# ugadiarov-la-phystech-edu/OCRL

Hardware: AMD Instinct MI355X
Metric: images/sec (node) SLATE pretrain 128x128, 6 slots, 3 iters (higher is better)
Workload: dtype f32

## Files before the change

ocrl_amd/csrc/slot_attn.hip:

```cpp
#include "common.h"
#include "kernels.h"

#define SA_C 64
#include <stdlib.h>
#define SA_TF 1024
#define SA_TB 512
#define SA_TLD 68
#define SA_WLD 17
#define SA_MAX_BLOCKS 2048

typedef float f32x4_t __attribute__((ext_vector_type(4)));
#define MFMA16(a, b, c) __builtin_amdgcn_mfma_f32_16x16x4f32((a), (b), (c), 0, 0, 0)

__device__ inline float sigmoidf_(float x) { return 1.0f / (1.0f + __expf(-x)); }
#define SA_ROR(v, n) __builtin_bit_cast(float, __builtin_amdgcn_update_dpp(0, __builtin_bit_cast(int, (v)), 0x120 + (n), 0xF, 0xF, false))
__device__ inline float red16_sum(float v) {
    v += SA_ROR(v, 8); v += SA_ROR(v, 4); v += SA_ROR(v, 2); v += SA_ROR(v, 1);
    return v;
}
__device__ inline float red16_max(float v) {
    v = fmaxf(v, SA_ROR(v, 8)); v = fmaxf(v, SA_ROR(v, 4)); v = fmaxf(v, SA_ROR(v, 2)); v = fmaxf(v, SA_ROR(v, 1));
    return v;
}
__device__ inline float redg_sum(float v) {
// ... 601 lines not shown
            for (int c = 0; c < 4; ++c) od[c] = pos0 < N ? dxb[pos0 * 16 + 4 * c + g] : make_float4(0.f, 0.f, 0.f, 0.f);
        }
        f32x4_t L = (f32x4_t){l0, l0, l0, l0}, DA = (f32x4_t){d0, d0, d0, d0};
#pragma unroll
        for (int k = 0; k < 16; ++k) { L = MFMA16(xn[k], qpr[k], L); DA = MFMA16(xn[k], dur[k], DA); }
#pragma unroll
        for (int c = 0; c < 4; ++c)
            *reinterpret_cast<float4*>(tile + li * SA_TLD + 16 * c + 4 * g) = make_float4(xn[4 * c], xn[4 * c + 1], xn[4 * c + 2], xn[4 * c + 3]);
        f32x4_t dl, wn;
#pragma unroll
        for (int r = 0; r < 4; ++r) {
            const float x = li < K ? L[r] : -INFINITY;
            const float mx = red16_max(x);
            const float e = li < K ? __expf(x - mx) : 0.f;
            const float a = e / red16_sum(e);
            const float da = (DA[r] - udv) * icv;
            const float dot = red16_sum(a * da);
            const bool ok = li < K && (t * 16 + 4 * g + r) < N;
            dl[r] = ok ? a * (da - dot) : 0.f;
            wn[r] = ok ? (a + eps) * icv : 0.f;
            sdl += dl[r];
            wt0[(4 * g + r) * SA_WLD + li] = wn[r];
            wt1[(4 * g + r) * SA_WLD + li] = dl[r];
        }
        __builtin_amdgcn_wave_barrier();
#pragma unroll
        for (int r = 0; r < 4; ++r)
#pragma unroll
            for (int m = 0; m < 4; ++m) acc[m] = MFMA16(tile[(4 * g + r) * SA_TLD + 16 * m + li], dl[r], acc[m]);
        f32x4_t Dx[4];
#pragma unroll
        for (int m = 0; m < 4; ++m) Dx[m] = (f32x4_t){0.f, 0.f, 0.f, 0.f};
#pragma unroll
        for (int s = 0; s < NS; ++s) {
            const float wa = wt0[li * SA_WLD + 4 * s + g], da2 = wt1[li * SA_WLD + 4 * s + g];
#pragma unroll
            for (int m = 0; m < 4; ++m) { Dx[m] = MFMA16(wa, duB[s][m], Dx[m]); Dx[m] = MFMA16(da2, qpB[s][m], Dx[m]); }
        }
        __builtin_amdgcn_wave_barrier();
#pragma unroll
        for (int m = 0; m < 4; ++m)
#pragma unroll
            for (int r = 0; r < 4; ++r) tile[(4 * g + r) * SA_TLD + 16 * m + li] = Dx[m][r];
        __builtin_amdgcn_wave_barrier();
        float dv[16];
#pragma unroll
        for (int c = 0; c < 4; ++c) {
            const float4 d4 = *reinterpret_cast<const float4*>(tile + li * SA_TLD + 16 * c + 4 * g);
            dv[4 * c] = d4.x; dv[4 * c + 1] = d4.y; dv[4 * c + 2] = d4.z; dv[4 * c + 3] = d4.w;
        }
        __builtin_amdgcn_wave_barrier();
        const int pos = t * 16 + li;
        if (!FIRST) {
#pragma unroll
            for (int c = 0; c < 4; ++c) { dv[4 * c] += od[c].x; dv[4 * c + 1] += od[c].y; dv[4 * c + 2] += od[c].z; dv[4 * c + 3] += od[c].w; }
        }
        if (FINAL) {
            float m1 = 0.f, m2 = 0.f;
#pragma unroll
            for (int k = 0; k < 16; ++k) { m1 += dv[k]; m2 += dv[k] * xn[k]; }
            m1 = redg_sum(m1) * (1.0f / SA_C);
            m2 = redg_sum(m2) * (1.0f / SA_C);
#pragma unroll
            for (int k = 0; k < 16; ++k) dv[k] = rs * (dv[k] - m1 - xn[k] * m2);
        }
        if (pos < N) {
#pragma unroll
            for (int c = 0; c < 4; ++c) dxb[pos * 16 + 4 * c + g] = make_float4(dv[4 * c], dv[4 * c + 1], dv[4 * c + 2], dv[4 * c + 3]);
        }
#pragma unroll
        for (int c = 0; c < 4; ++c) cur[c] = nxt[c];
    }
    sdl = redg_sum(sdl);
    __syncthreads();
    if (li < K) {
#pragma unroll
        for (int m = 0; m < 4; ++m)
#pragma unroll
            for (int r = 0; r < 4; ++r) scr[(wv * K + li) * (SA_C + 1) + 16 * m + 4 * g + r] = acc[m][r];
        if (g == 0) scr[(wv * K + li) * (SA_C + 1) + SA_C] = sdl;
    }
}

template <int K, bool FIRST, bool FINAL>
__device__ __forceinline__ void sa_stream_bwd2(const float4* __restrict__ xb, float4* __restrict__ dxb, int N, const float* qg, const float* qb,
                                               const float* dug, const float* dub, const float* cs, const float* ud, float eps, float* tiles,
                                               float* scr, int tile0, int tile1) {
    const int tid = threadIdx.x, lane = tid & 63, wv = tid >> 6, nw = blockDim.x >> 6, li = lane & 15, g = lane >> 4;
    float* tile = tiles + wv * (16 * SA_TLD + 2 * 16 * SA_WLD);
    float* wt = tile + 16 * SA_TLD;
    float qpr[16], dur[16];
#pragma unroll
    for (int k = 0; k < 16; ++k) {
        const int ch = 16 * (k >> 2) + 4 * g + (k & 3);
        qpr[k] = li < K ? qg[li * SA_C + ch] * SA_LOG2E : 0.f;
        dur[k] = li < K ? dug[li * SA_C + ch] : 0.f;
    }
    float duA[4][4], qgA[4][4];
#pragma unroll
    for (int m = 0; m < 4; ++m)
#pragma unroll
        for (int r = 0; r < 4; ++r) {
            const int slot = 4 * g + r;
            duA[m][r] = slot < K ? dug[slot * SA_C + 16 * m + li] : 0.f;
            qgA[m][r] = slot < K ? qg[slot * SA_C + 16 * m + li] : 0.f;
        }
    float qbr[4], dbr[4], icr[4];
#pragma unroll
    for (int r = 0; r < 4; ++r) {
        const int slot = 4 * g + r;
        qbr[r] = slot < K ? qb[slot] * SA_LOG2E : -1e30f;
        icr[r] = slot < K ? 1.0f / cs[slot] : 0.f;
        dbr[r] = slot < K ? dub[slot] - ud[slot] : 0.f;
    }
    f32x4_t acc[4];
#pragma unroll
    for (int m = 0; m < 4; ++m) acc[m] = (f32x4_t){0.f, 0.f, 0.f, 0.f};
    float sdl[4] = {0.f, 0.f, 0.f, 0.f};
    const int ntile = tile1;
    float4 cur[4];
    if (tile0 + wv < ntile) sa_load_tile(xb, N, tile0 + wv, li, g, cur);
#pragma unroll 1
    for (int t = tile0 + wv; t < ntile; t += nw) {
        float4 nxt[4];
        if (t + nw < ntile) sa_load_tile(xb, N, t + nw, li, g, nxt);
        const int pos = t * 16 + li;
        float4 od[4];
        if (!FIRST) {
#pragma unroll
            for (int c = 0; c < 4; ++c) od[c] = pos < N ? dxb[pos * 16 + 4 * c + g] : make_float4(0.f, 0.f, 0.f, 0.f);
        }
        f32x2_t v2[8];
#pragma unroll
        for (int c = 0; c < 4; ++c) { v2[2 * c] = (f32x2_t){cur[c].x, cur[c].y}; v2[2 * c + 1] = (f32x2_t){cur[c].z, cur[c].w}; }
        f32x2_t s2 = ((v2[0] + v2[1]) + (v2[2] + v2[3])) + ((v2[4] + v2[5]) + (v2[6] + v2[7]));
        const float mu = sa_xrow_sum4(s2.x + s2.y) * (1.0f / SA_C);
        const f32x2_t mu2 = (f32x2_t){mu, mu};
#pragma unroll
        for (int k = 0; k < 8; ++k) v2[k] -= mu2;
        f32x2_t q2 = v2[0] * v2[0];
#pragma unroll
        for (int k = 1; k < 8; ++k) q2 = __builtin_elementwise_fma(v2[k], v2[k], q2);
        const float rs = __builtin_amdgcn_rsqf(sa_xrow_sum4(q2.x + q2.y) * (1.0f / SA_C) + 1e-5f);
        f32x4_t La = (f32x4_t){0.f, 0.f, 0.f, 0.f}, Lb = La, Da = La, Db = La;
#pragma unroll
        for (int k = 0; k < 8; ++k) {
            La = MFMA16(qpr[2 * k], v2[k].x, La);
            Da = MFMA16(dur[2 * k], v2[k].x, Da);
            Lb = MFMA16(qpr[2 * k + 1], v2[k].y, Lb);
            Db = MFMA16(dur[2 * k + 1], v2[k].y, Db);
        }
#pragma unroll
        for (int c = 0; c < 4; ++c)
            *reinterpret_cast<float4*>(tile + li * SA_TLD + 16 * c + 4 * g) = make_float4(v2[2 * c].x, v2[2 * c].y, v2[2 * c + 1].x, v2[2 * c + 1].y);
        float l[4];
#pragma unroll
        for (int r = 0; r < 4; ++r) l[r] = __builtin_fmaf(La[r] + Lb[r], rs, qbr[r]);
        float mx = fmaxf(fmaxf(l[0], l[1]), fmaxf(l[2], l[3]));
        mx = sa_xrow16(mx, true);
        if (K > 8) mx = sa_xrow32(mx, true);
        float a[4];
#pragma unroll
        for (int r = 0; r < 4; ++r) a[r] = __builtin_amdgcn_exp2f(l[r] - mx);
        float sm = (a[0] + a[1]) + (a[2] + a[3]);
        sm = sa_xrow16(sm, false);
        if (K > 8) sm = sa_xrow32(sm, false);
        const float inv = __builtin_amdgcn_rcpf(sm);
        float da[4], dot = 0.f;
#pragma unroll
        for (int r = 0; r < 4; ++r) {
            a[r] *= inv;
            da[r] = (__builtin_fmaf(Da[r] + Db[r], rs, dbr[r])) * icr[r];
            dot = __builtin_fmaf(a[r], da[r], dot);
        }
        dot = sa_xrow16(dot, false);
        if (K > 8) dot = sa_xrow32(dot, false);
        const float live = pos < N ? 1.f : 0.f;
        float dl[4], wn[4];
#pragma unroll
        for (int r = 0; r < 4; ++r) {
            dl[r] = a[r] * (da[r] - dot) * live;
            wn[r] = (a[r] + eps) * icr[r] * live;
            sdl[r] += dl[r];
            wt[(4 * g + r) * SA_WT_LD + li] = dl[r] * rs;
        }
        __builtin_amdgcn_wave_barrier();
        const float4 wb4 = *reinterpret_cast<const float4*>(wt + li * SA_WT_LD + 4 * g);
        const float wb[4] = {wb4.x, wb4.y, wb4.z, wb4.w};
#pragma unroll
        for (int r = 0; r < 4; ++r)
#pragma unroll
            for (int m = 0; m < 4; ++m) acc[m] = MFMA16(tile[(4 * g + r) * SA_TLD + 16 * m + li], wb[r], acc[m]);
        f32x4_t Dx[4];
#pragma unroll
        for (int m = 0; m < 4; ++m) Dx[m] = (f32x4_t){0.f, 0.f, 0.f, 0.f};
#pragma unroll
        for (int r = 0; r < 4; ++r)
#pragma unroll
            for (int m = 0; m < 4; ++m) {
                Dx[m] = MFMA16(duA[m][r], wn[r], Dx[m]);
                Dx[m] = MFMA16(qgA[m][r], dl[r], Dx[m]);
            }
        __builtin_amdgcn_wave_barrier();
        float dv[16];
#pragma unroll
        for (int m = 0; m < 4; ++m) { dv[4 * m] = Dx[m][0]; dv[4 * m + 1] = Dx[m][1]; dv[4 * m + 2] = Dx[m][2]; dv[4 * m + 3] = Dx[m][3]; }
        if (!FIRST) {
#pragma unroll
            for (int c = 0; c < 4; ++c) { dv[4 * c] += od[c].x; dv[4 * c + 1] += od[c].y; dv[4 * c + 2] += od[c].z; dv[4 * c + 3] += od[c].w; }
        }
        if (FINAL) {
            float m1 = 0.f, m2 = 0.f;
#pragma unroll
            for (int k = 0; k < 8; ++k) {
                m1 += dv[2 * k] + dv[2 * k + 1];
                m2 += dv[2 * k] * v2[k].x + dv[2 * k + 1] * v2[k].y;
            }
            m1 = sa_xrow_sum4(m1) * (1.0f / SA_C);
            m2 = sa_xrow_sum4(m2) * rs * (1.0f / SA_C);
#pragma unroll
            for (int k = 0; k < 8; ++k) {
                dv[2 * k] = rs * (dv[2 * k] - m1 - v2[k].x * rs * m2);
                dv[2 * k + 1] = rs * (dv[2 * k + 1] - m1 - v2[k].y * rs * m2);
            }
        }
        if (pos < N) {
#pragma unroll
            for (int c = 0; c < 4; ++c) dxb[pos * 16 + 4 * c + g] = make_float4(dv[4 * c], dv[4 * c + 1], dv[4 * c + 2], dv[4 * c + 3]);
        }
#pragma unroll
        for (int c = 0; c < 4; ++c) cur[c] = nxt[c];
    }
#pragma unroll
    for (int r = 0; r < 4; ++r) sdl[r] = red16_sum(sdl[r]);
    __syncthreads();
    if (li < K) {
#pragma unroll
        for (int m = 0; m < 4; ++m)
#pragma unroll
            for (int r = 0; r < 4; ++r) scr[(wv * K + li) * (SA_C + 1) + 16 * m + 4 * g + r] = acc[m][r];
    }
    if (li == 0) {
#pragma unroll
        for (int r = 0; r < 4; ++r)
            if (4 * g + r < K) scr[(wv * K + 4 * g + r) * (SA_C + 1) + SA_C] = sdl[r];
    }
}

template <int K, int G>
struct SaBwdLds {
    float *ds, *t2, *t0, *t1, *dgi, *dgh, *dhid, *qp, *dup, *dqp, *qg, *dug, *cs, *ud, *qb, *dub, *sdl, *gacc;
    __device__ SaBwdLds(float* sm, int D, int H, int NH) {
        constexpr int C = SA_C, KB = SaGeo<K, G>::KB, KP = SaGeo<K, G>::KP;
        const int KV = NH * KP;
        ds = sm;
        t2 = ds + KP * D;
        t0 = t2 + KP * D;
        t1 = t0 + KB * D;
        dgi = t1 + KB * D;
        dgh = dgi + KB * 3 * D;
        dhid = dgh + KB * 3 * D;
        qp = dhid + KB * H;
        dup = qp + KV * C;
        dqp = dup + KV * C;
        qg = dqp + KV * C;
        dug = qg + KV * C;
        cs = dug + KV * C;
        ud = cs + 16;
        qb = ud + 16;
        dub = qb + 16;
        sdl = dub + 16;
        gacc = sdl + 16;
    }
};

template <int K, int G>
__device__ __forceinline__ void sa_bwd_part1(const SaBwdLds<K, G>& L, const SlotAttnArgs& p, const SaWts& wo, const SaSave& so, const SaGrad& go,
                                             const SaRowMap& sv, const SaRowMap& gr, int nvalid) {
    constexpr int C = SA_C, NB = SaGeo<K, G>::NB, KB = SaGeo<K, G>::KB, KP = SaGeo<K, G>::KP;
    const int D = p.D, H = p.H, tid = threadIdx.x, nt = blockDim.x, NH = p.NH, dh = D / NH, KV = NH * KP;
    const float* W = p.wts;
    float* dg_m = L.gacc + 2 * D;  float* db_m = L.gacc + 3 * D;
#pragma unroll 1
    for (int hb = 0; hb < NB; ++hb) {
        const int j0 = hb * KB, kv = (nvalid - j0) < KB ? (nvalid - j0 > 0 ? nvalid - j0 : 0) : KB;
// ... 38 lines not shown
#pragma unroll 1
        for (int h = 0; h < NH; ++h)
            matvec<KB>(W + wo.WvT, D / 16, 0, h * dh / 16, dh, C, t1 + h * dh, D, L.dup + (h * KP + j0) * C, C, nullptr, 1.f);
    }
    for (int h = 0; h < NH; ++h) rows_get(L.qp + h * KP * C, sv, so.qp + h * C, 0, nvalid, C);
    for (int i = tid; i < KV * C; i += nt)
        if (((i >> 6) % KP) >= nvalid) { L.qp[i] = 0.f; L.dup[i] = 0.f; }
    __syncthreads();
    if (tid < KV) {
        const int h = tid / KP, r = tid - h * KP;
        if (r < nvalid) {
            const float* row = sv(r);
            L.cs[tid] = row[so.csum + h];
            float a = 0.f;
            for (int c = 0; c < C; ++c) a += row[so.up + h * C + c] * L.dup[tid * C + c];
            L.ud[tid] = a;
        }
    }
    __syncthreads();
    sa_fold_affine(L.qp, W + wo.ln_in_g, W + wo.ln_in_b, L.qg, L.qb, KV);
    sa_fold_affine(L.dup, W + wo.ln_in_g, W + wo.ln_in_b, L.dug, L.dub, KV);
    __syncthreads();
}

template <int K, int G>
__device__ __forceinline__ void sa_bwd_part2(const SaBwdLds<K, G>& L, const SlotAttnArgs& p, const SaWts& wo, const SaSave& so, const SaGrad& go,
                                             const SaRowMap& sv, const SaRowMap& gr, int b0, int NS, int nvalid) {
    constexpr int C = SA_C, NB = SaGeo<K, G>::NB, KB = SaGeo<K, G>::KB, KP = SaGeo<K, G>::KP;
    const int D = p.D, tid = threadIdx.x, nt = blockDim.x, NH = p.NH, dh = D / NH, KV = NH * KP;
    const float* W = p.wts;
    float* dg_s = L.gacc;  float* db_s = L.gacc + D;
    float* dg_in = L.gacc + 4 * D;  float* db_in = L.gacc + 4 * D + C;
    float *dqp = L.dqp, *sdl = L.sdl, *t0 = L.t0, *t1 = L.t1;
    const int pstride = NH * K * (C + 1);
    if (tid < KV) {
        const int h = tid / KP, r = tid - h * KP;
        sdl[tid] = r < nvalid ? sa_psum(p.parts + (size_t)(b0 + r / K) * NS * pstride, NS, pstride, (h * K + r % K) * (C + 1) + C) : 0.f;
    }
    for (int i = tid; i < KV * C; i += nt) {
        const int v = i >> 6, c = i & 63, h = v / KP, r = v - h * KP;
        dqp[i] = r < nvalid ? sa_psum(p.parts + (size_t)(b0 + r / K) * NS * pstride, NS, pstride, (h * K + r % K) * (C + 1) + c) : 0.f;
    }
    __syncthreads();
    if (tid < C) {
        float dg = 0.f, db = 0.f;
        for (int h = 0; h < NH; ++h)
            for (int r = 0; r < nvalid; ++r) {
                const int j = h * KP + r;
                dg += L.dup[j * C + tid] * sv(r)[so.upn + h * C + tid] + L.qp[j * C + tid] * dqp[j * C + tid];
                db += L.dup[j * C + tid] + L.qp[j * C + tid] * sdl[j];
            }
        dg_in[tid] += dg;
        db_in[tid] += db;
    }
    __syncthreads();
    for (int i = tid; i < KV * C; i += nt) {
        const int j = i >> 6, c = i & 63;
        if ((j % KP) < nvalid) dqp[i] = dqp[i] * W[wo.ln_in_g + c] + W[wo.ln_in_b + c] * sdl[j];
    }
    __syncthreads();
    for (int h = 0; h < NH; ++h) rows_put(dqp + h * KP * C, gr, go.qp + h * C, 0, nvalid, C);
#pragma unroll 1
    for (int hb = 0; hb < NB; ++hb) {
        const int j0 = hb * KB, kv = (nvalid - j0) < KB ? (nvalid - j0 > 0 ? nvalid - j0 : 0) : KB;
        float* dsB = L.ds + j0 * D;
#pragma unroll 1
        for (int h = 0; h < NH; ++h)
            matvec<KB>(W + wo.Wk, C / 16, h * dh / 16, 0, C, dh, dqp + (h * KP + j0) * C, C, t1 + h * dh, D, nullptr, p.scale);
        rows_put(t1, gr, go.q, j0, kv, D);
        rows_get(t0, sv, so.sprev, j0, kv, D);
        for (int i = kv * D + tid; i < KB * D; i += nt) t0[i] = 0.f;
        matvec<KB>(W + wo.WqT, D / 16, 0, 0, D, D, t1, D, dsB, D, nullptr, 1.f);
        for (int i = tid; i < kv * D; i += nt) { t1[i] = dsB[i]; dsB[i] = L.t2[j0 * D + i]; }
        __syncthreads();
        ln_rows_bwd(t1, t0, dsB, 1, W + wo.ln_s_g, dg_s, db_s, kv, D);
        __syncthreads();
    }
}

__host__ __device__ inline size_t sa_xchg_bwd_floats(int K, int D) {
    const int KI = K > 8 ? 2 * ((K + 1) / 2) : K;
    return ((size_t)KI * D + 3 * (size_t)KI * SA_C + 64 + 15) & ~(size_t)15;
}
template <int K, int G>
__global__ __launch_bounds__(SA_TB) void sa_slot_bwd_kernel(SlotAttnArgs p, SaWts wo, SaSave so, SaGrad go, int t_hi, int t_lo, int NS) {
    extern __shared__ __attribute__((aligned(16))) float sm[];
    const int D = p.D;
    constexpr int C = SA_C, KP = SaGeo<K, G>::KP;
    const int nt = blockDim.x, tid = threadIdx.x, NH = p.NH, KV = NH * KP, KI = sa_ki(NH * K);
    const SaBwdLds<K, G> L(sm, D, p.H, NH);
    const int b0 = blockIdx.x * G;
    const int nimg = (p.B - b0) < G ? (p.B - b0) : G, nvalid = nimg * K;
    const size_t XF = sa_xchg_bwd_floats(NH * K, D);
    float* xg0 = p.xchg + (size_t)b0 * XF;
    const int SM = 4 * D + 2 * C;
    float* gs = p.g_small + (size_t)b0 * SM;
    if (t_hi < 0) {
        for (int i = tid; i < KP * D; i += nt) L.ds[i] = i < nvalid * D ? p.dslots[(size_t)b0 * K * D + i] : 0.f;
        for (int i = tid; i < SM; i += nt) L.gacc[i] = 0.f;
    } else {
        for (int i = tid; i < KP * D; i += nt) { const int r = i / D, c = i - r * D; L.t2[i] = r < nvalid ? xg0[(size_t)(r / K) * XF + (r % K) * D + c] : 0.f; }
        for (int i = tid; i < KV * C; i += nt) {
            const int v = i >> 6, c = i & 63, h = v / KP, r = v - h * KP;
            L.dup[i] = r < nvalid ? xg0[(size_t)(r / K) * XF + KI * D + (h * K + r % K) * C + c] : 0.f;
        }
        for (int i = tid; i < SM; i += nt) L.gacc[i] = gs[i];
        for (int h = 0; h < NH; ++h) rows_get(L.qp + h * KP * C, sa_rows(p.save, so.ld, b0, t_hi, p.I, K), so.qp + h * C, 0, nvalid, C);
        for (int i = tid; i < KV * C; i += nt)
            if (((i >> 6) % KP) >= nvalid) L.qp[i] = 0.f;
    }
    __syncthreads();
    if (t_hi >= 0)
        sa_bwd_part2<K, G>(L, p, wo, so, go, sa_rows(p.save, so.ld, b0, t_hi, p.I, K), sa_rows(p.grows, go.ld, b0, t_hi, p.I, K), b0, NS, nvalid);
    if (t_lo >= 0) {
        sa_bwd_part1<K, G>(L, p, wo, so, go, sa_rows(p.save, so.ld, b0, t_lo, p.I, K), sa_rows(p.grows, go.ld, b0, t_lo, p.I, K), nvalid);
        for (int i = tid; i < nvalid * D; i += nt) { const int r = i / D, c = i - r * D; xg0[(size_t)(r / K) * XF + (r % K) * D + c] = L.t2[i]; }
        for (int i = tid; i < KV * C; i += nt) {
            const int v = i >> 6, c = i & 63, h = v / KP, r = v - h * KP;
            if (r >= nvalid) continue;
            float* x = xg0 + (size_t)(r / K) * XF + KI * D + (h * K + r % K) * C + c;
            x[0] = L.dup[i]; x[KI * C] = L.qg[i]; x[2 * KI * C] = L.dug[i];
        }
        if (tid < KV) {
            const int h = tid / KP, r = tid - h * KP;
            if (r < nvalid) {
                float* x = xg0 + (size_t)(r / K) * XF + KI * D + 3 * KI * C + h * K + r % K;
                x[0] = L.qb[tid]; x[16] = L.dub[tid]; x[32] = L.cs[tid]; x[48] = L.ud[tid];
            }
        }
    } else {
        for (int i = tid; i < nvalid * D; i += nt) p.dslots0[(size_t)b0 * K * D + i] = L.ds[i];
    }
    for (int i = tid; i < SM; i += nt) gs[i] = L.gacc[i];
    for (int i = tid; i < (nimg - 1) * SM; i += nt) gs[SM + i] = 0.f;
}
template <int K, bool FIRST, bool FINAL, bool V2>
__global__ __launch_bounds__(SA_TS, 2) void sa_stream_bwd_kernel(SlotAttnArgs p, int NS) {
    extern __shared__ __attribute__((aligned(16))) float sm[];
    constexpr int C = SA_C, KP = SaBlk<K>::KP;
    const int D = p.D, N = p.N, nt = blockDim.x, nw = nt >> 6, tid = threadIdx.x;
    float* qg = sm;
    float* dug = qg + KP * C;
    float* sv4 = dug + KP * C;
    float* tiles = sv4 + 64;
    const int b = blockIdx.x / NS, h = blockIdx.x % NS;
    const float* xg = p.xchg + (size_t)b * sa_xchg_bwd_floats(K, D);
    const float *g_qg = xg + KP * D + KP * C, *g_dug = g_qg + KP * C, *g_small4 = g_dug + KP * C;
    for (int i = tid; i < K * C; i += nt) { qg[i] = g_qg[i]; dug[i] = g_dug[i]; }
    if (tid < 64) sv4[tid] = g_small4[tid];
    __syncthreads();
    const float4* xb = reinterpret_cast<const float4*>(p.x + (size_t)b * N * C);
    float4* dxb = reinterpret_cast<float4*>(p.dx + (size_t)b * N * C);
    const int ntile = (N + 15) / 16, per = (ntile + NS - 1) / NS;
    const int t0 = h * per, t1 = (t0 + per < ntile) ? t0 + per : ntile;
    if (V2) sa_stream_bwd2<K, FIRST, FINAL>(xb, dxb, N, qg, sv4, dug, sv4 + 16, sv4 + 32, sv4 + 48, p.eps, tiles, tiles, t0, t1 > t0 ? t1 : t0);
    else sa_stream_bwd<K, FIRST, FINAL>(xb, dxb, N, qg, sv4, dug, sv4 + 16, sv4 + 32, sv4 + 48, p.eps, tiles, tiles, t0, t1 > t0 ? t1 : t0);
    __syncthreads();
    float* part = p.parts + ((size_t)b * NS + h) * K * (C + 1);
    for (int i = tid; i < K * (C + 1); i += nt) {
        float a = 0.f;
        for (int w = 0; w < nw; ++w) a += tiles[w * K * (C + 1) + i];
        part[i] = a;
    }
}

static size_t sa_fwd_smem(int K, int G, int D, int H, int NH = 1) {
    const int NB = K > 8 ? 2 : 1, KB = K > 8 ? (K + 1) / 2 : G * K, KP = NB * KB;
    return (size_t)(KP * D + KB * D * 3 + KB * 3 * D * 2 + KB * H + NH * KP * SA_C * 3 + 32) * 4;
}
static size_t sa_bwd_smem(int K, int G, int D, int H, int NH = 1) {
    const int NB = K > 8 ? 2 : 1, KB = K > 8 ? (K + 1) / 2 : G * K, KP = NB * KB;
    return (size_t)(KP * D * 2 + KB * D * 2 + KB * 3 * D * 2 + KB * H + NH * KP * SA_C * 5 + 80 + 4 * D + 2 * SA_C) * 4;
}
#define SA_LDS_MAX (160 * 1024 - 256)
int sa_plan(int K, int D, int H, int NH, SaPlan* pl) {
    OCRL_REQUIRE(K >= 1 && K <= 16, "slot_attn: 1 <= num_slots <= 16 supported (got %d)", K);
    OCRL_REQUIRE(D > 0 && H > 0 && D % 64 == 0 && H % 64 == 0 && D <= 256 && H <= 256,
                 "slot_attn: slot/mlp size must be multiples of 64, <= 256 (got %d / %d)", D, H);
    OCRL_REQUIRE(NH >= 1 && D % NH == 0, "slot_attn: the slot size %d does not divide into %d heads", D, NH);
    if (NH > 1)
        OCRL_REQUIRE(K <= 8 && NH * K <= 16 && (D / NH) % 16 == 0,
                     "slot_attn: with %d heads, heads * num_slots <= 16 and a head width that is a multiple of 16 are supported (num_slots %d, slot size %d)", NH, K, D);
    int G = 1;
    if (NH == 1 && K <= 8 && 16 / K > 1) {
        static int gmode = -1;
        if (gmode < 0) { const char* e = getenv("OCRL_SA_GROUP"); gmode = e ? atoi(e) : 1; }
        const int GM = 16 / K;
        if (gmode && sa_fwd_smem(K, GM, D, H) <= SA_LDS_MAX && sa_bwd_smem(K, GM, D, H) <= SA_LDS_MAX) G = GM;
    }
    pl->G = G; pl->NB = K > 8 ? 2 : 1; pl->KB = K > 8 ? (K + 1) / 2 : G * K; pl->KS = NH * K;
    pl->smem_fwd = sa_fwd_smem(K, G, D, H, NH); pl->smem_bwd = sa_bwd_smem(K, G, D, H, NH);
    OCRL_REQUIRE(pl->smem_fwd <= SA_LDS_MAX && pl->smem_bwd <= SA_LDS_MAX, "slot_attn: LDS request %zu / %zu too large (num_slots %d, heads %d, slot size %d, mlp size %d)",
                 pl->smem_fwd, pl->smem_bwd, K, NH, D, H);
    return 0;
}
size_t sa_xchg_floats_host(int K, int D) {
    const size_t f = sa_xchg_floats(K, D), g = sa_xchg_bwd_floats(K, D);
    return f > g ? f : g;
}
size_t sa_parts_floats_host(int B, int K) { return (size_t)(SA_MAX_BLOCKS + B) * K * (SA_C + 1); }

static int sa_splits(int B, int N, int per_cu) {
    static int ncu = 0, mult = 0;
    if (!ncu) {
        int dev = 0;
        hipDeviceProp_t prop;
        ncu = (hipGetDevice(&dev) == hipSuccess && hipGetDeviceProperties(&prop, dev) == hipSuccess) ? prop.multiProcessorCount : 256;
        const char* e = getenv("OCRL_SA_WGS");
        mult = e ? atoi(e) : 0;
    }
    const int ntile = (N + 15) / 16;
    int target = (mult > 0 ? mult : per_cu) * ncu;
    if (target > SA_MAX_BLOCKS) target = SA_MAX_BLOCKS;
    int ns = B <= target ? target / B : 1;
    if (const char* f = getenv("OCRL_SA_NS")) { const int v = atoi(f); if (v > 0 && (long long)B * v <= SA_MAX_BLOCKS) ns = v; }
    if (ns > ntile / 8) ns = ntile / 8;
    return ns < 1 ? 1 : ns;
}

template <int K, int G>
static int sa_launch_kg(const SlotAttnArgs& a, const SaPlan& pl, int backward, hipStream_t st) {
    constexpr int KP = SaBlk<K>::KP;
    static_assert(SaGeo<K, G>::NB == (K > 8 ? 2 : 1) && SaGeo<K, G>::KB == (K > 8 ? (K + 1) / 2 : G * K), "sa_plan states the kernels' geometry");
    const size_t smem = backward ? pl.smem_bwd : pl.smem_fwd;
    static_assert((SA_TS / 64) * 16 * SA_TLD >= (SA_TS / 64) * 16 * (SA_C + 1), "streaming workgroup: partial scratch must fit the tile region");
    const SaWts wo = sa_wts_layout(a.C, a.D, a.H);
    const SaSave so = sa_save_layout(a.C, a.D, a.H);
    const SaGrad go = sa_grad_layout(a.C, a.D, a.H);
    static size_t attr_f = 0, attr_b = 0;
    if (!backward && smem > attr_f) {
        OCRL_HIP(hipFuncSetAttribute((const void*)sa_slot_fwd_kernel<K, G>, hipFuncAttributeMaxDynamicSharedMemorySize, (int)smem));
        attr_f = smem;
    }
    if (backward && smem > attr_b) {
        OCRL_HIP(hipFuncSetAttribute((const void*)sa_slot_bwd_kernel<K, G>, hipFuncAttributeMaxDynamicSharedMemorySize, (int)smem));
        attr_b = smem;
    }
    static int fwd_form = -1;
    if (fwd_form < 0) { const char* e = getenv("OCRL_SA_FWD"); fwd_form = e ? atoi(e) : 2; }
    const int NS = sa_splits(a.B, a.N, backward ? 4 : (fwd_form == 1 ? 3 : 4));
    const int ngrp = (a.B + G - 1) / G;
    const int pi = prof_begin(backward ? PROF_SA_BWD : PROF_SA_FWD, st);
    if (!backward) {
        const size_t smem_stream = (size_t)(KP * SA_C + 16 + (SA_TS / 64) * (16 * SA_TLD + 16 * SA_WT_LD)) * 4;
        if (a.phase != 2) hipLaunchKernelGGL((sa_slot_fwd_kernel<K, G>), dim3(ngrp), dim3(SA_TF), smem, st, a, wo, so, -1, NS);
        for (int t = 0; t < a.I && a.phase != 1; ++t) {
            if (fwd_form == 1) hipLaunchKernelGGL((sa_stream_fwd_kernel<K, false>), dim3(a.B * NS), dim3(SA_TS), smem_stream, st, a, t, NS);
            else hipLaunchKernelGGL((sa_stream_fwd_kernel<K, true>), dim3(a.B * NS), dim3(SA_TS), smem_stream, st, a, t, NS);
            hipLaunchKernelGGL((sa_slot_fwd_kernel<K, G>), dim3(ngrp), dim3(SA_TF), smem, st, a, wo, so, t, NS);
        }
    } else {
        static int bwd_form = -1;
        if (bwd_form < 0) { const char* e = getenv("OCRL_SA_BWD"); bwd_form = e ? atoi(e) : 2; }
        static_assert(16 * SA_WT_LD <= 2 * 16 * SA_WLD, "the weight patch of the second form must fit the first form's two patches");
        const size_t smem_stream = (size_t)(2 * KP * SA_C + 64 + (SA_TS / 64) * (16 * SA_TLD + 2 * 16 * SA_WLD)) * 4;
        hipLaunchKernelGGL((sa_slot_bwd_kernel<K, G>), dim3(ngrp), dim3(SA_TB), smem, st, a, wo, so, go, -1, a.I - 1, NS);
        for (int t = a.I - 1; t >= 0; --t) {
            const bool first = (t == a.I - 1), final_ = (t == 0);
            if (bwd_form == 1) {
                if (first && final_) hipLaunchKernelGGL((sa_stream_bwd_kernel<K, true, true, false>), dim3(a.B * NS), dim3(SA_TS), smem_stream, st, a, NS);
                else if (first) hipLaunchKernelGGL((sa_stream_bwd_kernel<K, true, false, false>), dim3(a.B * NS), dim3(SA_TS), smem_stream, st, a, NS);
                else if (final_) hipLaunchKernelGGL((sa_stream_bwd_kernel<K, false, true, false>), dim3(a.B * NS), dim3(SA_TS), smem_stream, st, a, NS);
                else hipLaunchKernelGGL((sa_stream_bwd_kernel<K, false, false, false>), dim3(a.B * NS), dim3(SA_TS), smem_stream, st, a, NS);
            } else {
                if (first && final_) hipLaunchKernelGGL((sa_stream_bwd_kernel<K, true, true, true>), dim3(a.B * NS), dim3(SA_TS), smem_stream, st, a, NS);
                else if (first) hipLaunchKernelGGL((sa_stream_bwd_kernel<K, true, false, true>), dim3(a.B * NS), dim3(SA_TS), smem_stream, st, a, NS);
                else if (final_) hipLaunchKernelGGL((sa_stream_bwd_kernel<K, false, true, true>), dim3(a.B * NS), dim3(SA_TS), smem_stream, st, a, NS);
                else hipLaunchKernelGGL((sa_stream_bwd_kernel<K, false, false, true>), dim3(a.B * NS), dim3(SA_TS), smem_stream, st, a, NS);
            }
            hipLaunchKernelGGL((sa_slot_bwd_kernel<K, G>), dim3(ngrp), dim3(SA_TB), smem, st, a, wo, so, go, t, t - 1, NS);
        }
    }
    prof_end(pi, st);
    OCRL_CHECK_LAUNCH("slot_attn");
    return 0;
}
typedef void (*SaStreamFwdFn)(SlotAttnArgs, int, int);
typedef void (*SaStreamBwdFn)(SlotAttnArgs, int);
template <int KS> static SaStreamBwdFn sa_stream_bwd_pick(bool first, bool final_) {
    if (first && final_) return sa_stream_bwd_kernel<KS, true, true, true>;
    if (first) return sa_stream_bwd_kernel<KS, true, false, true>;
    if (final_) return sa_stream_bwd_kernel<KS, false, true, true>;
    return sa_stream_bwd_kernel<KS, false, false, true>;
}
static SaStreamFwdFn sa_stream_fwd_fn(int KS) {
    switch (KS) {
#define SA_CASE(k) case k: return sa_stream_fwd_kernel<k, true>;
        SA_CASE(2) SA_CASE(3) SA_CASE(4) SA_CASE(5) SA_CASE(6) SA_CASE(7) SA_CASE(8) SA_CASE(9) SA_CASE(10) SA_CASE(11) SA_CASE(12) SA_CASE(13) SA_CASE(14) SA_CASE(15) SA_CASE(16)
#undef SA_CASE
    }
    return nullptr;
}
static SaStreamBwdFn sa_stream_bwd_fn(int KS, bool first, bool final_) {
    switch (KS) {
#define SA_CASE(k) case k: return sa_stream_bwd_pick<k>(first, final_);
        SA_CASE(2) SA_CASE(3) SA_CASE(4) SA_CASE(5) SA_CASE(6) SA_CASE(7) SA_CASE(8) SA_CASE(9) SA_CASE(10) SA_CASE(11) SA_CASE(12) SA_CASE(13) SA_CASE(14) SA_CASE(15) SA_CASE(16)
#undef SA_CASE
    }
    return nullptr;
}
__global__ void sa_attn_heads_sum_kernel(const float* __restrict__ in, float* __restrict__ out, long long rows, int K, int NH) {
    const long long n = rows * K;
    for (long long i = (long long)blockIdx.x * blockDim.x + threadIdx.x; i < n; i += (long long)gridDim.x * blockDim.x) {
        const long long r = i / K; const int k = (int)(i - r * K);
        float a = 0.f;
        for (int h = 0; h < NH; ++h) a += in[r * (NH * K) + h * K + k];
        out[i] = a;
    }
}
template <int K>
static int sa_launch_heads(const SlotAttnArgs& a0, const SaPlan& pl, int backward, hipStream_t st) {
    const int NH = a0.NH, KS = pl.KS, KPS = sa_ki(KS);
    const size_t smem = backward ? pl.smem_bwd : pl.smem_fwd;
    OCRL_REQUIRE(!a0.attn || a0.attn_heads, "slot_attn: the per-head attention scratch is missing");
    SlotAttnArgs a = a0;
    if (a.attn) a.attn = a0.attn_heads;
    const SaWts wo = sa_wts_layout(a.C, a.D, a.H);
    const SaSave so = sa_save_layout(a.C, a.D, a.H, NH);
    const SaGrad go = sa_grad_layout(a.C, a.D, a.H, NH);
    OCRL_HIP(hipFuncSetAttribute((const void*)(backward ? (const void*)sa_slot_bwd_kernel<K, 1> : (const void*)sa_slot_fwd_kernel<K, 1>),
                                 hipFuncAttributeMaxDynamicSharedMemorySize, (int)SA_LDS_MAX));
    const int NS = sa_splits(a.B, a.N, 4);
    const int pi = prof_begin(backward ? PROF_SA_BWD : PROF_SA_FWD, st);
    if (!backward) {
        const size_t smem_stream = (size_t)(KPS * SA_C + 16 + (SA_TS / 64) * (16 * SA_TLD + 16 * SA_WT_LD)) * 4;
        const SaStreamFwdFn fs = sa_stream_fwd_fn(KS);
        if (a.phase != 2) hipLaunchKernelGGL((sa_slot_fwd_kernel<K, 1>), dim3(a.B), dim3(SA_TF), smem, st, a, wo, so, -1, NS);
        for (int t = 0; t < a.I && a.phase != 1; ++t) {
            hipLaunchKernelGGL(fs, dim3(a.B * NS), dim3(SA_TS), smem_stream, st, a, t, NS);
            hipLaunchKernelGGL((sa_slot_fwd_kernel<K, 1>), dim3(a.B), dim3(SA_TF), smem, st, a, wo, so, t, NS);
        }
        if (a0.attn && a.phase != 1) {
            const long long rows = (long long)a.B * a.N;
            hipLaunchKernelGGL(sa_attn_heads_sum_kernel, dim3(cdiv(rows * K, 256) > 4096 ? 4096 : cdiv(rows * K, 256)), dim3(256), 0, st, a0.attn_heads, a0.attn, rows, K, NH);
        }
    } else {
        const size_t smem_stream = (size_t)(2 * KPS * SA_C + 64 + (SA_TS / 64) * (16 * SA_TLD + 2 * 16 * SA_WLD)) * 4;
        hipLaunchKernelGGL((sa_slot_bwd_kernel<K, 1>), dim3(a.B), dim3(SA_TB), smem, st, a, wo, so, go, -1, a.I - 1, NS);
        for (int t = a.I - 1; t >= 0; --t) {
            hipLaunchKernelGGL(sa_stream_bwd_fn(KS, t == a.I - 1, t == 0), dim3(a.B * NS), dim3(SA_TS), smem_stream, st, a, NS);
            hipLaunchKernelGGL((sa_slot_bwd_kernel<K, 1>), dim3(a.B), dim3(SA_TB), smem, st, a, wo, so, go, t, t - 1, NS);
        }
    }
    prof_end(pi, st);
    OCRL_CHECK_LAUNCH("slot_attn (heads)");
    return 0;
}

template <int K>
static int sa_launch_k(const SlotAttnArgs& a, const SaPlan& pl, int backward, hipStream_t st) {
    OCRL_REQUIRE(a.xchg && a.parts, "slot_attn: exchange / partial buffers missing");
    constexpr int GM = K <= 8 ? 16 / K : 1;
    if (GM > 1 && pl.G == GM) return sa_launch_kg<K, GM>(a, pl, backward, st);
    return sa_launch_kg<K, 1>(a, pl, backward, st);
}

int slot_attn_launch(const SlotAttnArgs& a, int backward, hipStream_t st) {
    OCRL_REQUIRE(a.C == SA_C, "slot_attn: input width must be %d (got %d)", SA_C, a.C);
    SaPlan pl;
    RC(sa_plan(a.K, a.D, a.H, a.NH, &pl));
    OCRL_REQUIRE(a.B > 0 && a.N > 0 && a.I >= 1, "slot_attn: empty problem");
    OCRL_REQUIRE((long long)a.N * 16 < (1ll << 31), "slot_attn: N too large for 32-bit row offsets");
    OCRL_REQUIRE(a.x && a.wts && ((uintptr_t)a.x & 15) == 0, "slot_attn: x/wts missing or x not 16-byte aligned");
    if (backward) OCRL_REQUIRE(a.dx && ((uintptr_t)a.dx & 15) == 0 && a.save && a.grows && a.dslots && a.dslots0 && a.g_small, "slot_attn bwd: missing buffers");
    else OCRL_REQUIRE(a.slots0 && a.slots, "slot_attn fwd: missing buffers");
    OCRL_REQUIRE(a.xchg && a.parts && ((uintptr_t)a.xchg & 15) == 0, "slot_attn: exchange / partial buffers missing or xchg not 16-byte aligned");
    if (a.NH > 1) {
        switch (a.K) {
#define SA_CASE(k) case k: return sa_launch_heads<k>(a, pl, backward, st);
            SA_CASE(1) SA_CASE(2) SA_CASE(3) SA_CASE(4) SA_CASE(5) SA_CASE(6) SA_CASE(7) SA_CASE(8)
#undef SA_CASE
        }
        return -1;
    }
    switch (a.K) {
#define SA_CASE(k) case k: return sa_launch_k<k>(a, pl, backward, st);
        SA_CASE(1) SA_CASE(2) SA_CASE(3) SA_CASE(4) SA_CASE(5) SA_CASE(6) SA_CASE(7) SA_CASE(8)
        SA_CASE(9) SA_CASE(10) SA_CASE(11) SA_CASE(12) SA_CASE(13) SA_CASE(14) SA_CASE(15) SA_CASE(16)
#undef SA_CASE
    }
    return -1;
}

__global__ void pack_kernel(const PackEntry* __restrict__ ent, float* __restrict__ dst) {
    const PackEntry e = ent[blockIdx.y];
    const int n = e.rows * e.cols;
    for (int i = blockIdx.x * blockDim.x + threadIdx.x; i < n; i += gridDim.x * blockDim.x) {
        if (e.transpose >= 2) {
            const int Et = e.transpose == 2 ? e.cols : e.rows, nks = Et >> 4;
            const int j = i & 3, lane = (i >> 2) & 63, rest = i >> 8, s = rest % nks, tile = rest / nks;
            const int col = tile * 16 + (lane & 15), k = s * 16 + (lane >> 4) * 4 + j;
            dst[e.dst_off + i] = e.transpose == 2 ? e.src[col * Et + k] : e.src[k * e.cols + col];
        } else if (e.transpose) {
            const int c = i / e.rows, r = i - c * e.rows;
            dst[e.dst_off + i] = e.src[r * e.cols + c];
        } else {
            dst[e.dst_off + i] = e.src[i];
        }
    }
}
int pack_launch(const PackEntry* entries_dev, int n_entries, int max_elems, float* dst, hipStream_t st) {
    int gx = cdiv(max_elems, 256);
    if (gx > 64) gx = 64;
    hipLaunchKernelGGL(pack_kernel, dim3(gx, n_entries), dim3(256), 0, st, entries_dev, dst);
    OCRL_CHECK_LAUNCH("pack");
    return 0;
}
```

Before: 1748.

## Defer slot-attention input gradient by recording per-iteration weights and replaying at end

Adds a new default backward form (OCRL_SA_BWD=3) for slot attention. Non-final iteration stream kernels no longer build and accumulate the full 64-channel dx per position. They store only compact per-slot attention weights (wn, dl) into the dx buffer, and the slot backward kernel saves that iteration's dug/qg into a history area. The final stream kernel reads those records and replays every iteration's contribution with extra MFMAs against the history held in LDS. This cuts dx read-modify-write traffic across iterations, at the cost of more LDS, extra MFMA work in the final pass, and a larger exchange buffer.

After: 1753 (median of 6 runs). About the same (+0.2%).

```diff
diff --git a/ocrl_amd/csrc/slot_attn.hip b/ocrl_amd/csrc/slot_attn.hip
--- a/ocrl_amd/csrc/slot_attn.hip
+++ b/ocrl_amd/csrc/slot_attn.hip
@@ -707,10 +707,24 @@
     }
 }
 
-template <int K, bool FIRST, bool FINAL>
+template <int K> struct SaRec {
+    static constexpr int NG = K > 8 ? 4 : 2;
+    static constexpr int Q = 2 * NG * 16;
+    static constexpr int MAXE = 256 / Q;
+    static constexpr int PER = K > 8 ? 1 : 2;
+    static constexpr int HOP = 2 * SA_C * SA_WT_LD;
+};
+template <int K>
+__device__ __forceinline__ int sa_rec_idx(bool whole, int j, int which, int g, int li) {
+    constexpr int NG = SaRec<K>::NG;
+    return whole ? j * SaRec<K>::Q + (which * NG + g) * 16 + li : li * 16 + j * 2 * NG + which * NG + g;
+}
+template <int K, bool FIRST, bool FINAL, bool REC = false>
 __device__ __forceinline__ void sa_stream_bwd2(const float4* __restrict__ xb, float4* __restrict__ dxb, int N, const float* qg, const float* qb,
                                                const float* dug, const float* dub, const float* cs, const float* ud, float eps, float* tiles,
-                                               float* scr, int tile0, int tile1) {
+                                               float* scr, int tile0, int tile1, int rec = 0, const float* hop = nullptr) {
+    static_assert(!REC || FIRST, "the record form never accumulates through dx");
+    constexpr bool DXN = !REC || FINAL;
     const int tid = threadIdx.x, lane = tid & 63, wv = tid >> 6, nw = blockDim.x >> 6, li = lane & 15, g = lane >> 4;
     float* tile = tiles + wv * (16 * SA_TLD + 2 * 16 * SA_WLD);
     float* wt = tile + 16 * SA_TLD;
@@ -722,14 +736,16 @@
         dur[k] = li < K ? dug[li * SA_C + ch] : 0.f;
     }
     float duA[4][4], qgA[4][4];
-#pragma unroll
-    for (int m = 0; m < 4; ++m)
-#pragma unroll
-        for (int r = 0; r < 4; ++r) {
-            const int slot = 4 * g + r;
-            duA[m][r] = slot < K ? dug[slot * SA_C + 16 * m + li] : 0.f;
-            qgA[m][r] = slot < K ? qg[slot * SA_C + 16 * m + li] : 0.f;
-        }
+    if (DXN) {
+#pragma unroll
+        for (int m = 0; m < 4; ++m)
+#pragma unroll
+            for (int r = 0; r < 4; ++r) {
+                const int slot = 4 * g + r;
+                duA[m][r] = slot < K ? dug[slot * SA_C + 16 * m + li] : 0.f;
+                qgA[m][r] = slot < K ? qg[slot * SA_C + 16 * m + li] : 0.f;
+            }
+    }
     float qbr[4], dbr[4], icr[4];
 #pragma unroll
     for (int r = 0; r < 4; ++r) {
@@ -743,6 +759,8 @@
     for (int m = 0; m < 4; ++m) acc[m] = (f32x4_t){0.f, 0.f, 0.f, 0.f};
     float sdl[4] = {0.f, 0.f, 0.f, 0.f};
     const int ntile = tile1;
+    constexpr int RPER = SaRec<K>::PER;
+    const int ngrp = REC && FINAL ? (rec + RPER - 1) / RPER : 0, ge = RPER == 2 ? g >> 1 : 0, gs = RPER == 2 ? g & 1 : g;
     float4 cur[4];
     if (tile0 + wv < ntile) sa_load_tile(xb, N, tile0 + wv, li, g, cur);
 #pragma unroll 1
@@ -750,6 +768,17 @@
         float4 nxt[4];
         if (t + nw < ntile) sa_load_tile(xb, N, t + nw, li, g, nxt);
         const int pos = t * 16 + li;
+        const bool whole = t * 16 + 16 <= N;
+        float4 rw[SaRec<K>::MAXE / RPER], rd[SaRec<K>::MAXE / RPER];
+        if (REC && FINAL) {
+#pragma unroll
+            for (int gi = 0; gi < SaRec<K>::MAXE / RPER; ++gi) {
+                const int j = gi * RPER + ge;
+                const bool have = gi < ngrp && j < rec && pos < N;
+                rw[gi] = have ? dxb[t * 256 + sa_rec_idx<K>(whole, j, 0, gs, li)] : make_float4(0.f, 0.f, 0.f, 0.f);
+                rd[gi] = have ? dxb[t * 256 + sa_rec_idx<K>(whole, j, 1, gs, li)] : make_float4(0.f, 0.f, 0.f, 0.f);
+            }
+        }
         float4 od[4];
         if (!FIRST) {
 #pragma unroll
@@ -816,6 +845,16 @@
         for (int r = 0; r < 4; ++r)
 #pragma unroll
             for (int m = 0; m < 4; ++m) acc[m] = MFMA16(tile[(4 * g + r) * SA_TLD + 16 * m + li], wb[r], acc[m]);
+        if (!DXN) {
+            __builtin_amdgcn_wave_barrier();
+            if (g < SaRec<K>::NG && pos < N) {
+                dxb[t * 256 + sa_rec_idx<K>(whole, rec, 0, g, li)] = make_float4(wn[0], wn[1], wn[2], wn[3]);
+                dxb[t * 256 + sa_rec_idx<K>(whole, rec, 1, g, li)] = make_float4(dl[0], dl[1], dl[2], dl[3]);
+            }
+#pragma unroll
+            for (int c = 0; c < 4; ++c) cur[c] = nxt[c];
+            continue;
+        }
         f32x4_t Dx[4];
 #pragma unroll
         for (int m = 0; m < 4; ++m) Dx[m] = (f32x4_t){0.f, 0.f, 0.f, 0.f};
@@ -826,6 +865,25 @@
                 Dx[m] = MFMA16(duA[m][r], wn[r], Dx[m]);
                 Dx[m] = MFMA16(qgA[m][r], dl[r], Dx[m]);
             }
+        if (REC) {
+#pragma unroll
+            for (int gi = 0; gi < SaRec<K>::MAXE / RPER; ++gi) {
+                if (gi >= ngrp) break;
+                const float* ha = hop + gi * SaRec<K>::HOP + li * SA_WT_LD + 4 * g;
+                const float bw[4] = {rw[gi].x, rw[gi].y, rw[gi].z, rw[gi].w}, bd[4] = {rd[gi].x, rd[gi].y, rd[gi].z, rd[gi].w};
+#pragma unroll
+                for (int m = 0; m < 4; ++m) {
+                    const float4 au = *reinterpret_cast<const float4*>(ha + 16 * m * SA_WT_LD);
+                    const float4 aq = *reinterpret_cast<const float4*>(ha + (SA_C + 16 * m) * SA_WT_LD);
+                    const float ua[4] = {au.x, au.y, au.z, au.w}, qa[4] = {aq.x, aq.y, aq.z, aq.w};
+#pragma unroll
+                    for (int r = 0; r < 4; ++r) {
+                        Dx[m] = MFMA16(ua[r], bw[r], Dx[m]);
+                        Dx[m] = MFMA16(qa[r], bd[r], Dx[m]);
+                    }
+                }
+            }
+        }
         __builtin_amdgcn_wave_barrier();
         float dv[16];
 #pragma unroll
@@ -1030,8 +1088,12 @@
     const int KI = K > 8 ? 2 * ((K + 1) / 2) : K;
     return ((size_t)KI * D + 3 * (size_t)KI * SA_C + 64 + 15) & ~(size_t)15;
 }
+__host__ __device__ inline size_t sa_xchg_hist_floats(int K) {
+    const int KI = K > 8 ? 2 * ((K + 1) / 2) : K;
+    return (size_t)(K > 8 ? 2 : 4) * 2 * KI * SA_C;
+}
 template <int K, int G>
-__global__ __launch_bounds__(SA_TB) void sa_slot_bwd_kernel(SlotAttnArgs p, SaWts wo, SaSave so, SaGrad go, int t_hi, int t_lo, int NS) {
+__global__ __launch_bounds__(SA_TB) void sa_slot_bwd_kernel(SlotAttnArgs p, SaWts wo, SaSave so, SaGrad go, int t_hi, int t_lo, int NS, float* hist) {
     extern __shared__ __attribute__((aligned(16))) float sm[];
     const int D = p.D;
     constexpr int C = SA_C, KP = SaGeo<K, G>::KP;
@@ -1068,6 +1130,10 @@
             if (r >= nvalid) continue;
             float* x = xg0 + (size_t)(r / K) * XF + KI * D + (h * K + r % K) * C + c;
             x[0] = L.dup[i]; x[KI * C] = L.qg[i]; x[2 * KI * C] = L.dug[i];
+            if (hist && t_lo >= 1) {
+                float* y = hist + ((size_t)(b0 + r / K) * sa_xchg_hist_floats(NH * K) + (size_t)(t_lo - 1) * 2 * KI * C) + (h * K + r % K) * C + c;
+                y[0] = L.dug[i]; y[KI * C] = L.qg[i];
+            }
         }
         if (tid < KV) {
             const int h = tid / KP, r = tid - h * KP;
@@ -1111,6 +1177,47 @@
         part[i] = a;
     }
 }
+template <int K, bool FINAL>
+__global__ __launch_bounds__(SA_TS, 2) void sa_stream_rec_kernel(SlotAttnArgs p, int NS, int t, const float* hist) {
+    extern __shared__ __attribute__((aligned(16))) float sm[];
+    constexpr int C = SA_C, KP = SaBlk<K>::KP, PER = SaRec<K>::PER, HOP = SaRec<K>::HOP;
+    const int D = p.D, N = p.N, nt = blockDim.x, nw = nt >> 6, tid = threadIdx.x;
+    float* qg = sm;
+    float* dug = qg + KP * C;
+    float* sv4 = dug + KP * C;
+    float* tiles = sv4 + 64;
+    float* hop = tiles + nw * (16 * SA_TLD + 2 * 16 * SA_WLD);
+    const int b = blockIdx.x / NS, h = blockIdx.x % NS;
+    const float* xg = p.xchg + (size_t)b * sa_xchg_bwd_floats(K, D);
+    const float *g_qg = xg + KP * D + KP * C, *g_dug = g_qg + KP * C, *g_small4 = g_dug + KP * C;
+    for (int i = tid; i < K * C; i += nt) { qg[i] = g_qg[i]; dug[i] = g_dug[i]; }
+    if (tid < 64) sv4[tid] = g_small4[tid];
+    const int nrec = FINAL ? p.I - 1 : t - 1;
+    if (FINAL) {
+        const float* hb = hist + (size_t)b * sa_xchg_hist_floats(K);
+        const int ngrp = (nrec + PER - 1) / PER;
+        for (int i = tid; i < ngrp * 2 * 16 * C; i += nt) {
+            const int ch = i & 63, k = (i >> 6) & 15, which = (i >> 10) & 1, gi = i >> 11;
+            const int e = PER == 2 ? 2 * gi + (k >> 3) : gi, slot = PER == 2 ? k & 7 : k;
+            hop[gi * HOP + (which * C + ch) * SA_WT_LD + k] = (e < nrec && slot < K) ? hb[((size_t)e * 2 + which) * KP * C + slot * C + ch] : 0.f;
+        }
+    }
+    __syncthreads();
+    const float4* xb = reinterpret_cast<const float4*>(p.x + (size_t)b * N * C);
+    float4* dxb = reinterpret_cast<float4*>(p.dx + (size_t)b * N * C);
+    const int ntile = (N + 15) / 16, per = (ntile + NS - 1) / NS;
+    const int t0 = h * per, t1 = (t0 + per < ntile) ? t0 + per : ntile;
+    sa_stream_bwd2<K, true, FINAL, true>(xb, dxb, N, qg, sv4, dug, sv4 + 16, sv4 + 32, sv4 + 48, p.eps, tiles, tiles, t0, t1 > t0 ? t1 : t0, nrec, hop);
+    __syncthreads();
+    float* part = p.parts + ((size_t)b * NS + h) * K * (C + 1);
+    for (int i = tid; i < K * (C + 1); i += nt) {
+        float a = 0.f;
+        for (int w = 0; w < nw; ++w) a += tiles[w * K * (C + 1) + i];
+        part[i] = a;
+    }
+}
+static bool sa_rec_fits(int K, int I) { return I >= 2 && I - 1 <= (K > 8 ? 2 : 4); }
+static size_t sa_rec_hop_floats(int K, int I) { const int per = K > 8 ? 1 : 2; return (size_t)((I - 1 + per - 1) / per) * 2 * SA_C * SA_WT_LD; }
 
 static size_t sa_fwd_smem(int K, int G, int D, int H, int NH = 1) {
     const int NB = K > 8 ? 2 : 1, KB = K > 8 ? (K + 1) / 2 : G * K, KP = NB * KB;
@@ -1142,9 +1249,12 @@
                  pl->smem_fwd, pl->smem_bwd, K, NH, D, H);
     return 0;
 }
-size_t sa_xchg_floats_host(int K, int D) {
+static size_t sa_xchg_state_floats(int K, int D) {
     const size_t f = sa_xchg_floats(K, D), g = sa_xchg_bwd_floats(K, D);
     return f > g ? f : g;
+}
+size_t sa_xchg_floats_host(int K, int D) {
+    return sa_xchg_state_floats(K, D) + sa_xchg_hist_floats(K);
 }
 size_t sa_parts_floats_host(int B, int K) { return (size_t)(SA_MAX_BLOCKS + B) * K * (SA_C + 1); }
 
@@ -1166,6 +1276,11 @@
     return ns < 1 ? 1 : ns;
 }
 
+static int sa_bwd_form() {
+    static int form = -1;
+    if (form < 0) { const char* e = getenv("OCRL_SA_BWD"); form = e ? atoi(e) : 3; }
+    return form;
+}
 template <int K, int G>
 static int sa_launch_kg(const SlotAttnArgs& a, const SaPlan& pl, int backward, hipStream_t st) {
     constexpr int KP = SaBlk<K>::KP;
@@ -1198,14 +1313,18 @@
             hipLaunchKernelGGL((sa_slot_fwd_kernel<K, G>), dim3(ngrp), dim3(SA_TF), smem, st, a, wo, so, t, NS);
         }
     } else {
-        static int bwd_form = -1;
-        if (bwd_form < 0) { const char* e = getenv("OCRL_SA_BWD"); bwd_form = e ? atoi(e) : 2; }
+        const int bwd_form = sa_bwd_form();
         static_assert(16 * SA_WT_LD <= 2 * 16 * SA_WLD, "the weight patch of the second form must fit the first form's two patches");
         const size_t smem_stream = (size_t)(2 * KP * SA_C + 64 + (SA_TS / 64) * (16 * SA_TLD + 2 * 16 * SA_WLD)) * 4;
-        hipLaunchKernelGGL((sa_slot_bwd_kernel<K, G>), dim3(ngrp), dim3(SA_TB), smem, st, a, wo, so, go, -1, a.I - 1, NS);
+        const bool rec = bwd_form == 3 && sa_rec_fits(K, a.I);
+        float* hist = rec ? a.xchg + (size_t)a.B * sa_xchg_state_floats(K, a.D) : nullptr;
+        hipLaunchKernelGGL((sa_slot_bwd_kernel<K, G>), dim3(ngrp), dim3(SA_TB), smem, st, a, wo, so, go, -1, a.I - 1, NS, hist);
         for (int t = a.I - 1; t >= 0; --t) {
             const bool first = (t == a.I - 1), final_ = (t == 0);
-            if (bwd_form == 1) {
+            if (rec) {
+                if (final_) hipLaunchKernelGGL((sa_stream_rec_kernel<K, true>), dim3(a.B * NS), dim3(SA_TS), smem_stream + sa_rec_hop_floats(K, a.I) * 4, st, a, NS, t, hist);
+                else hipLaunchKernelGGL((sa_stream_rec_kernel<K, false>), dim3(a.B * NS), dim3(SA_TS), smem_stream, st, a, NS, t, hist);
+            } else if (bwd_form == 1) {
                 if (first && final_) hipLaunchKernelGGL((sa_stream_bwd_kernel<K, true, true, false>), dim3(a.B * NS), dim3(SA_TS), smem_stream, st, a, NS);
                 else if (first) hipLaunchKernelGGL((sa_stream_bwd_kernel<K, true, false, false>), dim3(a.B * NS), dim3(SA_TS), smem_stream, st, a, NS);
                 else if (final_) hipLaunchKernelGGL((sa_stream_bwd_kernel<K, false, true, false>), dim3(a.B * NS), dim3(SA_TS), smem_stream, st, a, NS);
@@ -1216,7 +1335,7 @@
                 else if (final_) hipLaunchKernelGGL((sa_stream_bwd_kernel<K, false, true, true>), dim3(a.B * NS), dim3(SA_TS), smem_stream, st, a, NS);
                 else hipLaunchKernelGGL((sa_stream_bwd_kernel<K, false, false, true>), dim3(a.B * NS), dim3(SA_TS), smem_stream, st, a, NS);
             }
-            hipLaunchKernelGGL((sa_slot_bwd_kernel<K, G>), dim3(ngrp), dim3(SA_TB), smem, st, a, wo, so, go, t, t - 1, NS);
+            hipLaunchKernelGGL((sa_slot_bwd_kernel<K, G>), dim3(ngrp), dim3(SA_TB), smem, st, a, wo, so, go, t, t - 1, NS, hist);
         }
     }
     prof_end(pi, st);
@@ -1225,6 +1344,7 @@
 }
 typedef void (*SaStreamFwdFn)(SlotAttnArgs, int, int);
 typedef void (*SaStreamBwdFn)(SlotAttnArgs, int);
+typedef void (*SaStreamRecFn)(SlotAttnArgs, int, int, const float*);
 template <int KS> static SaStreamBwdFn sa_stream_bwd_pick(bool first, bool final_) {
     if (first && final_) return sa_stream_bwd_kernel<KS, true, true, true>;
     if (first) return sa_stream_bwd_kernel<KS, true, false, true>;
@@ -1242,6 +1362,14 @@
 static SaStreamBwdFn sa_stream_bwd_fn(int KS, bool first, bool final_) {
     switch (KS) {
 #define SA_CASE(k) case k: return sa_stream_bwd_pick<k>(first, final_);
+        SA_CASE(2) SA_CASE(3) SA_CASE(4) SA_CASE(5) SA_CASE(6) SA_CASE(7) SA_CASE(8) SA_CASE(9) SA_CASE(10) SA_CASE(11) SA_CASE(12) SA_CASE(13) SA_CASE(14) SA_CASE(15) SA_CASE(16)
+#undef SA_CASE
+    }
+    return nullptr;
+}
+static SaStreamRecFn sa_stream_rec_fn(int KS, bool final_) {
+    switch (KS) {
+#define SA_CASE(k) case k: return final_ ? sa_stream_rec_kernel<k, true> : sa_stream_rec_kernel<k, false>;
         SA_CASE(2) SA_CASE(3) SA_CASE(4) SA_CASE(5) SA_CASE(6) SA_CASE(7) SA_CASE(8) SA_CASE(9) SA_CASE(10) SA_CASE(11) SA_CASE(12) SA_CASE(13) SA_CASE(14) SA_CASE(15) SA_CASE(16)
 #undef SA_CASE
     }
@@ -1284,10 +1412,13 @@
         }
     } else {
         const size_t smem_stream = (size_t)(2 * KPS * SA_C + 64 + (SA_TS / 64) * (16 * SA_TLD + 2 * 16 * SA_WLD)) * 4;
-        hipLaunchKernelGGL((sa_slot_bwd_kernel<K, 1>), dim3(a.B), dim3(SA_TB), smem, st, a, wo, so, go, -1, a.I - 1, NS);
+        const bool rec = sa_bwd_form() == 3 && sa_rec_fits(KS, a.I);
+        float* hist = rec ? a.xchg + (size_t)a.B * sa_xchg_state_floats(KS, a.D) : nullptr;
+        hipLaunchKernelGGL((sa_slot_bwd_kernel<K, 1>), dim3(a.B), dim3(SA_TB), smem, st, a, wo, so, go, -1, a.I - 1, NS, hist);
         for (int t = a.I - 1; t >= 0; --t) {
-            hipLaunchKernelGGL(sa_stream_bwd_fn(KS, t == a.I - 1, t == 0), dim3(a.B * NS), dim3(SA_TS), smem_stream, st, a, NS);
-            hipLaunchKernelGGL((sa_slot_bwd_kernel<K, 1>), dim3(a.B), dim3(SA_TB), smem, st, a, wo, so, go, t, t - 1, NS);
+            if (rec) hipLaunchKernelGGL(sa_stream_rec_fn(KS, t == 0), dim3(a.B * NS), dim3(SA_TS), smem_stream + (t == 0 ? sa_rec_hop_floats(KS, a.I) * 4 : 0), st, a, NS, t, hist);
+            else hipLaunchKernelGGL(sa_stream_bwd_fn(KS, t == a.I - 1, t == 0), dim3(a.B * NS), dim3(SA_TS), smem_stream, st, a, NS);
+            hipLaunchKernelGGL((sa_slot_bwd_kernel<K, 1>), dim3(a.B), dim3(SA_TB), smem, st, a, wo, so, go, t, t - 1, NS, hist);
         }
     }
     prof_end(pi, st);
```
